# andreeaiana/manner

Measured on AMD Instinct MI355X. Metric: candidate news encoded+scored/sec, higher is better.
Workload: dtype f16; 1 GPU; configs[1]: CR-Module late fusion, MIND-small shape (65238-news pool), bert-base-uncased architectu~; modules=1, parallelism=dp1 (impressions sharded, no collective)

## Files before the change

### manner_amd/csrc/attention.hip

```cpp
#include <math.h>
#include <stdlib.h>

#include "common.h"

namespace manner {
namespace {

template <typename TE, int NKT>
__device__ __forceinline__ void attn_wave_bf16(const TE* __restrict__ qkv, TE* __restrict__ ctx,
                                               int tok0, int L, int H, int head, char* vl) {
  typedef typename E16<TE>::v8 e16x8;
  typedef typename E16<TE>::v4 e16x4;
  const int lane = threadIdx.x & 63, rr = lane & 31, h = lane >> 5;
  char* ol = vl + NKT * 32 * 128;
  const size_t ld = 3 * (size_t)H;
  const TE* Qb = qkv + (size_t)tok0 * ld + head * 64;
  const TE* Kb = Qb + H;
  const TE* Vb = Qb + 2 * H;

  const int r8 = lane >> 3, c8 = lane & 7;
  f32x4 kt_[NKT][4], qt_[4];
#pragma unroll
  for (int kt = 0; kt < NKT; ++kt)
#pragma unroll
// ... 874 lines not shown
        Row8<T>::load(Vb + (size_t)min(key, L - 1) * ld, vr);
#pragma unroll
        for (int e = 0; e < 8; ++e) o[e] = fmaf(p, vr[e], o[e]);
      }
    }
  }
  sum += __shfl_xor(sum, 8, 64); sum += __shfl_xor(sum, 16, 64); sum += __shfl_xor(sum, 32, 64);
#pragma unroll
  for (int e = 0; e < 8; ++e) {
    o[e] += __shfl_xor(o[e], 8, 64); o[e] += __shfl_xor(o[e], 16, 64); o[e] += __shfl_xor(o[e], 32, 64);
  }
  if (g == 0) {
    const float inv = 1.0f / sum;
#pragma unroll
    for (int e = 0; e < 8; ++e) o[e] *= inv;
    Row8<T>::store(dst, o);
  }
}

template <typename T>
__global__ __launch_bounds__(256) void attn_cls_kernel(const T* __restrict__ qcls, const T* __restrict__ kv,
                                                       T* __restrict__ ctx, const int32_t* __restrict__ cu,
                                                       int64_t n_pairs, int heads, int H) {
  const int64_t pair = (int64_t)blockIdx.x * 4 + (threadIdx.x >> 6);
  if (pair >= n_pairs) return;
  const int lane = threadIdx.x & 63, g = lane >> 3, c = lane & 7;
  const int n = (int)(pair / heads), head = (int)(pair - (int64_t)n * heads);
  const int tok0 = cu[n], L = cu[n + 1] - tok0;
  const size_t ld = 2 * (size_t)H;
  const T* Kb = kv + (size_t)tok0 * ld + head * 64 + 8 * c;
  const T* Vb = Kb + H;
  float q[8];
  Row8<T>::load(qcls + (size_t)n * H + head * 64 + 8 * c, q);
  if (L > MANNER_HIP_MAX_LEN) {
    attn_cls_long<T>(Kb, Vb, q, L, ld, g, ctx + (size_t)n * H + head * 64 + 8 * c);
    return;
  }
  constexpr int MAXR = MANNER_HIP_MAX_LEN / 8;
  float sc[MAXR];
  float mx = -INFINITY;
#pragma unroll
  for (int r = 0; r < MAXR; ++r) {
    const int key = 8 * r + g;
    float s = -INFINITY;
    if (8 * r < L) {
      float kr[8];
      Row8<T>::load(Kb + (size_t)min(key, L - 1) * ld, kr);
      float d = 0.f;
#pragma unroll
      for (int e = 0; e < 8; ++e) d = fmaf(q[e], kr[e], d);
      d += __shfl_xor(d, 1, 64); d += __shfl_xor(d, 2, 64); d += __shfl_xor(d, 4, 64);
      s = key < L ? d * 0.125f : -INFINITY;
    }
    sc[r] = s;
    mx = fmaxf(mx, s);
  }
  mx = fmaxf(mx, __shfl_xor(mx, 8, 64)); mx = fmaxf(mx, __shfl_xor(mx, 16, 64)); mx = fmaxf(mx, __shfl_xor(mx, 32, 64));
  float sum = 0.f, o[8] = {0.f, 0.f, 0.f, 0.f, 0.f, 0.f, 0.f, 0.f};
#pragma unroll
  for (int r = 0; r < MAXR; ++r) {
    if (8 * r < L) {
      const int key = 8 * r + g;
      const float p = expf(sc[r] - mx);
      sum += p;
      float vr[8];
      Row8<T>::load(Vb + (size_t)min(key, L - 1) * ld, vr);
#pragma unroll
      for (int e = 0; e < 8; ++e) o[e] = fmaf(p, vr[e], o[e]);
    }
  }
  sum += __shfl_xor(sum, 8, 64); sum += __shfl_xor(sum, 16, 64); sum += __shfl_xor(sum, 32, 64);
#pragma unroll
  for (int e = 0; e < 8; ++e) {
    o[e] += __shfl_xor(o[e], 8, 64); o[e] += __shfl_xor(o[e], 16, 64); o[e] += __shfl_xor(o[e], 32, 64);
  }
  if (g == 0) {
    const float inv = 1.0f / sum;
#pragma unroll
    for (int e = 0; e < 8; ++e) o[e] *= inv;
    Row8<T>::store(ctx + (size_t)n * H + head * 64 + 8 * c, o);
  }
}

}

int attention_cls(DType dt, const void* qcls, const void* kv, void* ctx_cls, const int32_t* cu, int64_t n_news, int heads,
                  int H, hipStream_t stream) {
  if (H != heads * 64) return fail(MANNER_HIP_E_INVALID, "head_dim must be 64 (H=%d heads=%d)", H, heads);
  const int64_t pairs = n_news * heads;
  dim3 g((unsigned)((pairs + 3) / 4)), b(256);
  if (dt == DT_BF16)
    hipLaunchKernelGGL(attn_cls_kernel<bf16_t>, g, b, 0, stream, static_cast<const bf16_t*>(qcls), static_cast<const bf16_t*>(kv),
                       static_cast<bf16_t*>(ctx_cls), cu, pairs, heads, H);
  else if (dt == DT_F16)
    hipLaunchKernelGGL(attn_cls_kernel<f16_t>, g, b, 0, stream, static_cast<const f16_t*>(qcls), static_cast<const f16_t*>(kv),
                       static_cast<f16_t*>(ctx_cls), cu, pairs, heads, H);
  else
    hipLaunchKernelGGL(attn_cls_kernel<float>, g, b, 0, stream, static_cast<const float*>(qcls), static_cast<const float*>(kv),
                       static_cast<float*>(ctx_cls), cu, pairs, heads, H);
  MANNER_LAUNCH_CHECK();
  return MANNER_HIP_OK;
}

static int attention_long(DType dt, const void* qkv, void* ctx, const int32_t* cu, int64_t pairs, int heads, int H, int max_len,
                          hipStream_t stream, void* split_out, DType split_dt) {
  if (is_16bit(dt)) {
    const int n_qb = (max_len + 32 * LONG16_WAVES - 1) / (32 * LONG16_WAVES);
    const int rows_cap = (max_len + 31) / 32 * 32;
    const int lds = rows_cap * 256 + LONG16_WAVES * 4096;
    static bool lds_raised_dev[MAX_DEVICES] = {};
    bool& lds_raised = lds_raised_dev[current_device_slot()];
    if (!lds_raised) {
      const int cap = MANNER_HIP_MAX_LEN_INFER * 256 + LONG16_WAVES * 4096;
      MANNER_HIP_TRY(hipFuncSetAttribute(reinterpret_cast<const void*>(attn_long16_kernel<bf16_t>), hipFuncAttributeMaxDynamicSharedMemorySize, cap));
      MANNER_HIP_TRY(hipFuncSetAttribute(reinterpret_cast<const void*>(attn_long16_kernel<f16_t>), hipFuncAttributeMaxDynamicSharedMemorySize, cap));
      lds_raised = true;
    }
    const dim3 grid((unsigned)(pairs * n_qb)), block(64 * LONG16_WAVES);
    if (dt == DT_F16)
      hipLaunchKernelGGL(attn_long16_kernel<f16_t>, grid, block, lds, stream, static_cast<const f16_t*>(qkv), static_cast<f16_t*>(ctx), cu,
                         pairs, n_qb, heads, H, rows_cap);
    else
      hipLaunchKernelGGL(attn_long16_kernel<bf16_t>, grid, block, lds, stream, static_cast<const bf16_t*>(qkv), static_cast<bf16_t*>(ctx), cu,
                         pairs, n_qb, heads, H, rows_cap);
  } else {
    const int n_qb = (max_len + 32 * LONGF_WAVES - 1) / (32 * LONGF_WAVES);
    static bool lds_raised_dev[MAX_DEVICES] = {};
    bool& lds_raised = lds_raised_dev[current_device_slot()];
    if (!lds_raised) {
      MANNER_HIP_TRY(hipFuncSetAttribute(reinterpret_cast<const void*>(attn_long_f32_kernel), hipFuncAttributeMaxDynamicSharedMemorySize, LONGF_LDS));
      lds_raised = true;
    }
    hipLaunchKernelGGL(attn_long_f32_kernel, dim3((unsigned)(pairs * n_qb)), dim3(64 * LONGF_WAVES), LONGF_LDS, stream,
                       static_cast<const float*>(qkv), static_cast<float*>(ctx), cu, pairs, n_qb, heads, H, split_out, (int)split_dt);
  }
  MANNER_LAUNCH_CHECK();
  return MANNER_HIP_OK;
}

int attention_varlen(DType dt, const void* qkv, void* ctx, const int32_t* cu, int64_t n_news, int heads, int H,
                     int max_len, hipStream_t stream, void* split_out, DType split_dt) {
  if (H != heads * 64) return fail(MANNER_HIP_E_INVALID, "head_dim must be 64 (H=%d heads=%d)", H, heads);
  if (max_len < 1 || max_len > MANNER_HIP_MAX_LEN_INFER)
    return fail(MANNER_HIP_E_INVALID, "padded length %d outside [1, %d]", max_len, MANNER_HIP_MAX_LEN_INFER);
  const int64_t pairs = n_news * heads;
  const bool long_rows = max_len > MANNER_HIP_MAX_LEN;
  const int short_len = long_rows ? MANNER_HIP_MAX_LEN : max_len;
  if (is_16bit(dt)) {
    const int nkt = (short_len + 31) / 32;
    const int lds_per_wave = nkt * 32 * 128 + 4096;
    static bool lds_raised_dev[MAX_DEVICES] = {};
    bool& lds_raised = lds_raised_dev[current_device_slot()];
    if (!lds_raised) {
      MANNER_HIP_TRY(hipFuncSetAttribute(reinterpret_cast<const void*>(attn_bf16_kernel<bf16_t>), hipFuncAttributeMaxDynamicSharedMemorySize, 4 * (4 * 32 * 128 + 4096)));
      MANNER_HIP_TRY(hipFuncSetAttribute(reinterpret_cast<const void*>(attn_bf16_kernel<f16_t>), hipFuncAttributeMaxDynamicSharedMemorySize, 4 * (4 * 32 * 128 + 4096)));
      lds_raised = true;
    }
    if (dt == DT_F16)
      hipLaunchKernelGGL(attn_bf16_kernel<f16_t>, dim3((unsigned)((pairs + 3) / 4)), dim3(256), 4 * lds_per_wave, stream,
                         static_cast<const f16_t*>(qkv), static_cast<f16_t*>(ctx), cu, pairs, heads, H, lds_per_wave);
    else
      hipLaunchKernelGGL(attn_bf16_kernel<bf16_t>, dim3((unsigned)((pairs + 3) / 4)), dim3(256), 4 * lds_per_wave, stream,
                         static_cast<const bf16_t*>(qkv), static_cast<bf16_t*>(ctx), cu, pairs, heads, H, lds_per_wave);
  } else {
    static const bool valu = getenv("MANNER_HIP_ATTN_F32_VALU") != nullptr;
    if (valu) {
// ... 39 lines not shown
```

### manner_amd/csrc/common.h

```cpp
#pragma once
#include <hip/hip_runtime.h>
#include <stddef.h>
#include <stdint.h>

#include "manner_hip.h"

typedef __bf16 bf16_t;
typedef __bf16 bf16x8 __attribute__((ext_vector_type(8)));
typedef __bf16 bf16x4 __attribute__((ext_vector_type(4)));
typedef _Float16 f16_t;
typedef _Float16 f16x8 __attribute__((ext_vector_type(8)));
typedef _Float16 f16x4 __attribute__((ext_vector_type(4)));
typedef short s16x4 __attribute__((ext_vector_type(4)));
typedef float f32x16 __attribute__((ext_vector_type(16)));
typedef float f32x4 __attribute__((ext_vector_type(4)));

#define LDS_PTR(p) ((__attribute__((address_space(3))) void*)(p))
#define GLOBAL_PTR(p) ((const __attribute__((address_space(1))) void*)(p))

namespace manner {

int fail(int code, const char* fmt, ...);

#define MANNER_HIP_TRY(expr)                                                            \
// ... 28 lines not shown
                EPI_GELU_GRAD = 9 ,
                EPI_BIAS_GELU_DUAL16 = 10 ,
                EPI_GELU_GRAD16 = 11  };
enum DType { DT_F32 = 0, DT_BF16 = 1, DT_F16 = 2 };
static inline bool is_16bit(DType d) { return d != DT_F32; }

template <typename T> struct E16;
template <> struct E16<bf16_t> {
  typedef bf16x8 v8; typedef bf16x4 v4;
  static constexpr DType dtype = DT_BF16;
  static __device__ __forceinline__ f32x4 mfma16(const v8& a, const v8& b, const f32x4& c) { return __builtin_amdgcn_mfma_f32_16x16x32_bf16(a, b, c, 0, 0, 0); }
  static __device__ __forceinline__ f32x16 mfma32(const v8& a, const v8& b, const f32x16& c) { return __builtin_amdgcn_mfma_f32_32x32x16_bf16(a, b, c, 0, 0, 0); }
};
template <> struct E16<f16_t> {
  typedef f16x8 v8; typedef f16x4 v4;
  static constexpr DType dtype = DT_F16;
  static __device__ __forceinline__ f32x4 mfma16(const v8& a, const v8& b, const f32x4& c) { return __builtin_amdgcn_mfma_f32_16x16x32_f16(a, b, c, 0, 0, 0); }
  static __device__ __forceinline__ f32x16 mfma32(const v8& a, const v8& b, const f32x16& c) { return __builtin_amdgcn_mfma_f32_32x32x16_f16(a, b, c, 0, 0, 0); }
};

int gemm_tn(DType in, DType out, Epilogue epi, const void* X, const void* W, const float* bias,
            const void* residual, void* Y, int64_t m_bound, int N, int K, const int* m_total,
            hipStream_t stream);

int gemm_tn_batched16(DType in, const void* X, const void* W, const float* bias, float* Y, int batch, int64_t xs, int64_t ws,
                      int64_t ys, int rows, int N, int K, const int* m_total, hipStream_t stream);

struct DlnFinalize { void* mr_out; int32_t* arrive; float eps; bool done; };
int gemm_tn_dln(DType dt, Epilogue epi, const void* X, const void* W, const float* bias, const float* vec, const void* mr,
                void* part, void* Y, int64_t m_bound, int N, int K, const int* m_total, hipStream_t stream, int64_t m_exact = -1,
                DlnFinalize* fin = nullptr);

int pool_logits_mfma(const float* x, const float* W, const float* bias, const float* query, int64_t R, int D, int Q,
                     float* logits, hipStream_t stream);

bool pool_fused_supported(int64_t B, int64_t S, int D, int Q);
size_t pool_fused_workspace_bytes(int D, int Q);
int pool_fused(const float* x, const float* W, const float* bias, const float* query, int64_t B, int64_t S, int D, int Q, float* out,
               void* workspace, size_t workspace_bytes, hipStream_t stream);

int lengths_and_offsets(const int64_t* mask, int64_t n_news, int64_t padded_len, int32_t* lens,
                        int32_t* cu , int32_t* m_total , int64_t m_bound,
                        int64_t expect_tokens, int32_t* status, hipStream_t stream, int max_len);
int embed_layernorm(DType out, const int64_t* ids, int64_t n_news, int64_t padded_len, const int32_t* cu,
                    const float* word, const float* pos, const float* type0, const float* gamma,
                    const float* beta, int H, float eps, int pos_offset, int vocab, int max_pos,
                    void* x, int32_t* status, hipStream_t stream);
int layernorm_rows(DType out, const float* pre, const float* gamma, const float* beta, int H, float eps,
                   void* x, int64_t m_bound, const int* m_total, hipStream_t stream);
int embed_raw(DType dt, const int64_t* ids, int64_t n_news, int64_t padded_len, const int32_t* cu, const float* word,
              const float* pos, const float* type0, int H, float eps, int pos_offset, int vocab, int max_pos,
              void* raw, void* mr, int32_t* status, hipStream_t stream);
__device__ __forceinline__ float2 dln_row_stats(const float2 (&v)[16], float inv_h, float eps) {
  float s1 = v[0].x, s2 = v[0].y;
#pragma unroll
  for (int g = 1; g < 16; ++g) { s1 += v[g].x; s2 += v[g].y; }
  const float mean = s1 * inv_h;
  const float var = fmaxf(fmaf(s2, inv_h, -(mean * mean)), 0.f);
  return float2{mean, 1.0f / sqrtf(var + eps)};
}
int dln_finalize(const void* part, int groups, int H, float eps, void* mr, int64_t m_bound, const int* m_total,
                 hipStream_t stream);
int gather_cls_ln(DType dt, const void* raw, const void* mr, const int32_t* cu, int64_t n_news, int H, const float* gamma,
                  const float* beta, void* dst, hipStream_t stream);
int fold_layernorm(DType dt, const float* w, const float* bias, const float* gamma, const float* beta, int N, int K, void* wf,
                   float* c1, float* c2, hipStream_t stream);
int scatter_hidden(DType in, DType out_dt, const void* x, const void* mr, const int32_t* cu, int64_t n_news, int64_t lp, int H,
                   const float* gamma, const float* beta, void* out, hipStream_t stream);
int split3_rows(DType dt, bool weight, const float* x, void* out, int K, int64_t rows, const int* m_total, hipStream_t stream);
int layernorm_rows_split(DType split_dt, const float* pre, const float* gamma, const float* beta, int H, float eps, float* x, void* a3,
                         int64_t m_bound, const int* m_total, hipStream_t stream);
int add_vectors(const float* a, const float* b, float* out, int n, hipStream_t stream);
int set_device_int(int32_t* p, int32_t value, hipStream_t stream);
int gather_cls(DType in, const void* x, const int32_t* cu, int64_t n_news, int H, float* out, hipStream_t stream);
int gather_cls_rows(DType dt, const void* x, const int32_t* cu, int64_t n_news, int H, void* dst, hipStream_t stream);
int convert_f32_to_16(DType dt, const float* src, void* dst, int64_t n, hipStream_t stream);

int attention_varlen(DType dt, const void* qkv, void* ctx, const int32_t* cu, int64_t n_news, int heads,
                     int H, int max_len, hipStream_t stream, void* split_out = nullptr, DType split_dt = DT_F32);

int attention_cls(DType dt, const void* qcls, const void* kv, void* ctx_cls, const int32_t* cu, int64_t n_news,
                  int heads, int H, hipStream_t stream);

}
```

### manner_amd/csrc/encoder.hip

```cpp
#include <stdarg.h>
#include <stdio.h>
#include <stdlib.h>

#include <vector>

#include "common.h"

namespace manner {

static thread_local char g_err[512] = "";

int fail(int code, const char* fmt, ...) {
  va_list ap;
  va_start(ap, fmt);
  vsnprintf(g_err, sizeof(g_err), fmt, ap);
  va_end(ap);
  return code;
}

struct LayerWeights {
  void* wqkv = nullptr;
  void* wo = nullptr;
  void* w1 = nullptr;
  void* w2 = nullptr;
  void* wqkv_f = nullptr;
  void* w1_f = nullptr;
  float *cq1 = nullptr, *cf1 = nullptr;
};
struct LayerParams {
  float *bqkv, *bo, *ln1g, *ln1b, *b1, *b2, *ln2g, *ln2b;
  float *cq2 = nullptr, *cf2 = nullptr, *bo_res = nullptr, *b2_res = nullptr;
};

}

struct manner_hip_encoder {
  manner_hip_encoder_config cfg;
  uint32_t precisions = 0;
  float *word = nullptr, *pos = nullptr, *type0 = nullptr, *embg = nullptr, *embb = nullptr;
  std::vector<manner::LayerParams> params;
  std::vector<manner::LayerWeights> w[5];
  int32_t* status = nullptr;
  static constexpr int ARRIVE_CAP = 4096;
  int32_t* arrive = nullptr;
  std::vector<void*> allocs;
  int n_streams = 2;
  bool defer_ln = false;
  static constexpr int MAX_STREAMS = 4;
  hipStream_t side[MAX_STREAMS] = {};
  hipEvent_t join_ev[MAX_STREAMS] = {};
  hipEvent_t phase_ev[MAX_STREAMS] = {};
  bool profiling = false;
  struct Span { hipEvent_t a, b; int cls; };
  std::vector<Span> spans;
  std::vector<hipEvent_t> free_events;
};

namespace manner {
namespace {

inline DType act_dtype(int prec) { return prec == MANNER_HIP_PREC_BF16 ? DT_BF16 : prec == MANNER_HIP_PREC_F16 ? DT_F16 : DT_F32; }
inline size_t act_bytes(int prec) { return (prec == MANNER_HIP_PREC_BF16 || prec == MANNER_HIP_PREC_F16) ? 2 : 4; }
inline bool is_x3(int prec) { return prec == MANNER_HIP_PREC_BF16X3 || prec == MANNER_HIP_PREC_F16X3; }
inline DType x3_dtype(int prec) { return prec == MANNER_HIP_PREC_F16X3 ? DT_F16 : DT_BF16; }

int dev_alloc(manner_hip_encoder* e, size_t bytes, void** out) {
  MANNER_HIP_TRY(hipMalloc(out, bytes));
  e->allocs.push_back(*out);
  return MANNER_HIP_OK;
}
int dev_copy_f32(manner_hip_encoder* e, const float* src, size_t n, float** out, hipStream_t s) {
  int rc = dev_alloc(e, n * sizeof(float), (void**)out);
  if (rc) return rc;
  MANNER_HIP_TRY(hipMemcpyAsync(*out, src, n * sizeof(float), hipMemcpyDeviceToDevice, s));
  return MANNER_HIP_OK;
}
int pack_matrix(int prec, const float* src, size_t n, void* dst, size_t elem_off, hipStream_t s) {
  if (prec == MANNER_HIP_PREC_BF16 || prec == MANNER_HIP_PREC_F16)
    return convert_f32_to_16(prec == MANNER_HIP_PREC_F16 ? DT_F16 : DT_BF16, src, static_cast<char*>(dst) + elem_off * 2, (int64_t)n, s);
  MANNER_HIP_TRY(hipMemcpyAsync(static_cast<float*>(dst) + elem_off, src, n * sizeof(float), hipMemcpyDeviceToDevice, s));
  return MANNER_HIP_OK;
}

struct ProfScope {
  manner_hip_encoder* e; hipStream_t s; hipEvent_t a = nullptr, b = nullptr; int cls;
  static hipEvent_t get(manner_hip_encoder* e) {
    hipEvent_t ev = nullptr;
    if (!e->free_events.empty()) { ev = e->free_events.back(); e->free_events.pop_back(); }
    else if (hipEventCreate(&ev) != hipSuccess) ev = nullptr;
    return ev;
  }
  ProfScope(manner_hip_encoder* enc, hipStream_t st, int c) : e(enc), s(st), cls(c) {
    if (!e->profiling) return;
    a = get(e); b = get(e);
    if (a && b) (void)hipEventRecord(a, s);
  }
  ~ProfScope() {
    if (!a || !b) return;
    (void)hipEventRecord(b, s);
    e->spans.push_back({a, b, cls});
  }
};

struct Workspace {
  int32_t *lens, *cu, *m_total;
  float* pre;
  void *x, *qkv, *ctx, *ffn;
  void *xcls, *qcls;
  void *mr_in, *mr_mid, *part;
  int32_t* arrive = nullptr;
  void* a3;
  void* a3h;
  void *acc_x, *acc_ctx, *acc_x1;
  int32_t* cls_total;
  int64_t cls_cap;
};

constexpr int64_t CLS_CAP = 16384;

size_t carve(const manner_hip_encoder* e, int64_t max_news, int64_t m_cap, int prec, char* base, Workspace* ws) {
  const size_t es = act_bytes(prec);
  const size_t H = e->cfg.hidden, I = e->cfg.intermediate;
  size_t off = 0;
  if (ws) { ws->a3 = nullptr; ws->a3h = nullptr; }
  auto take = [&](size_t bytes) { size_t o = off; off += (size_t)round_up((int64_t)bytes, 256); return base ? base + o : nullptr; };
  char* p;
  p = take((size_t)max_news * 4); if (ws) ws->lens = (int32_t*)p;
  p = take((size_t)(max_news + 1) * 4); if (ws) ws->cu = (int32_t*)p;
  p = take(256); if (ws) ws->m_total = (int32_t*)p;
  p = take((size_t)m_cap * H * 4); if (ws) ws->pre = (float*)p;
  p = take((size_t)m_cap * H * es); if (ws) ws->x = p;
  p = take((size_t)m_cap * 3 * H * es); if (ws) ws->qkv = p;
  p = take((size_t)m_cap * H * es); if (ws) ws->ctx = p;
  p = take((size_t)m_cap * I * es); if (ws) ws->ffn = p;
  const size_t n_pad = (size_t)round_up(max_news, 256);
  p = take(n_pad * H * es); if (ws) ws->xcls = p;
  p = take(n_pad * H * es); if (ws) ws->qcls = p;
  p = take((size_t)m_cap * 8); if (ws) ws->mr_in = p;
  p = take((size_t)m_cap * 8); if (ws) ws->mr_mid = p;
  p = take((size_t)m_cap * (H / 64) * 8); if (ws) ws->part = p;
  if (is_x3(prec)) {
    p = take((size_t)m_cap * 3 * (H > I ? H : I) * 2); if (ws) ws->a3 = p;
    p = take((size_t)m_cap * 3 * H * 2); if (ws) ws->a3h = p;
  }
  const int64_t cls_cap = m_cap < CLS_CAP ? m_cap : CLS_CAP;
  if (ws) ws->cls_cap = cls_cap;
  p = take((size_t)(cls_cap + 256) * H * es); if (ws) ws->acc_x = p;
  p = take((size_t)(cls_cap + 256) * H * es); if (ws) ws->acc_ctx = p;
  p = take((size_t)(cls_cap + 256) * H * es); if (ws) ws->acc_x1 = p;
  p = take(256); if (ws) ws->cls_total = (int32_t*)p;
  return off;
}

struct PhaseGuard {
  hipEvent_t ev; hipStream_t s; bool done = false;
  void mark() { if (ev && !done) { (void)hipEventRecord(ev, s); done = true; } }
  ~PhaseGuard() { mark(); }
};

int encode_chunk(manner_hip_encoder* e, const int64_t* ids, const int64_t* mask, int64_t n_news, int64_t lp,
                 int64_t m_bound, int64_t expect_tokens, int prec, void* out, const Workspace& ws, hipStream_t s,
                 hipEvent_t phase_mark = nullptr, int hidden_layers = -1, DType hidden_dt = DT_F32, int64_t cls_off = 0) {
  PhaseGuard phase{phase_mark, s};
  const manner_hip_encoder_config& c = e->cfg;
  const DType dt = act_dtype(prec);
  const int H = c.hidden, I = c.intermediate;
  int rc;
  {
    ProfScope ps(e, s, MANNER_HIP_PROF_LENGTHS);
    if ((rc = lengths_and_offsets(mask, n_news, lp, ws.lens, ws.cu, ws.m_total, m_bound, expect_tokens, e->status, s,
                                 MANNER_HIP_MAX_LEN_INFER))) return rc;
  }
  const int pos_offset = c.arch == MANNER_HIP_ARCH_ROBERTA ? c.pad_id + 1 : 0;
#define PROF_STEP(cls, call) { ProfScope ps(e, s, cls); if ((rc = (call))) return rc; }
  const size_t es = act_bytes(prec);
  if (is_16bit(dt) && e->defer_ln) {
    PROF_STEP(MANNER_HIP_PROF_EMBED, embed_raw(dt, ids, n_news, lp, ws.cu, e->word, e->pos, e->type0, H, c.ln_eps, pos_offset,
                                               c.vocab, c.max_pos, ws.x, ws.mr_in, e->status, s))
    const int groups = H / 64;
    for (int l = 0; l < c.layers; ++l) {
      const LayerWeights& w = e->w[prec][l];
      const LayerParams& p = e->params[l];
      const float* g_in = l == 0 ? e->embg : e->params[l - 1].ln2g;
      const float* b_in = l == 0 ? e->embb : e->params[l - 1].ln2b;
      if (l == hidden_layers) break;
      if (hidden_layers < 0 && l + 1 == c.layers) {
        const int64_t n_bound = round_up(n_news, 256);
        const int32_t* n_total = ws.m_total + 1;
        const char* wkv = static_cast<const char*>(w.wqkv_f) + (size_t)H * H * 2;
        PROF_STEP(MANNER_HIP_PROF_GEMM_QKV, gemm_tn_dln(dt, EPI_NORM, ws.x, wkv, p.cq2 + H, w.cq1 + H, ws.mr_in, nullptr, ws.qkv, m_bound, 2 * H, H, ws.m_total, s, expect_tokens))
        char* ax = static_cast<char*>(ws.acc_x) + (size_t)cls_off * H * es;
        char* actx = static_cast<char*>(ws.acc_ctx) + (size_t)cls_off * H * es;
        PROF_STEP(MANNER_HIP_PROF_GATHER, gather_cls_ln(dt, ws.x, ws.mr_in, ws.cu, n_news, H, g_in, b_in, ax, s))
        PROF_STEP(MANNER_HIP_PROF_CLS_TAIL, gemm_tn(dt, dt, EPI_BIAS, ax, w.wqkv, p.bqkv, nullptr, ws.qcls, n_bound, H, H, n_total, s))
        PROF_STEP(MANNER_HIP_PROF_ATTENTION, attention_cls(dt, ws.qcls, ws.qkv, actx, ws.cu, n_news, c.heads, H, s))
        break;
      }
      PROF_STEP(MANNER_HIP_PROF_GEMM_QKV, gemm_tn_dln(dt, EPI_NORM, ws.x, w.wqkv_f, p.cq2, w.cq1, ws.mr_in, nullptr, ws.qkv, m_bound, 3 * H, H, ws.m_total, s, expect_tokens))
      PROF_STEP(MANNER_HIP_PROF_ATTENTION, attention_varlen(dt, ws.qkv, ws.ctx, ws.cu, n_news, c.heads, H, (int)lp, s))
      const bool fan_in = ws.arrive && m_bound / 192 + 1 <= manner_hip_encoder::ARRIVE_CAP;
      DlnFinalize fin_mid{ws.mr_mid, fan_in ? ws.arrive : nullptr, c.ln_eps, false}, fin_in{ws.mr_in, fan_in ? ws.arrive : nullptr, c.ln_eps, false};
      PROF_STEP(MANNER_HIP_PROF_GEMM_OUT, gemm_tn_dln(dt, EPI_NRES, ws.ctx, w.wo, p.bo_res, g_in, ws.mr_in, ws.part, ws.x, m_bound, H, H, ws.m_total, s, expect_tokens, &fin_mid))
      if (!fin_mid.done) PROF_STEP(MANNER_HIP_PROF_LAYERNORM, dln_finalize(ws.part, groups, H, c.ln_eps, ws.mr_mid, m_bound, ws.m_total, s))
      if (l == 0) phase.mark();
      PROF_STEP(MANNER_HIP_PROF_GEMM_FFN1, gemm_tn_dln(dt, EPI_NORM_GELU, ws.x, w.w1_f, p.cf2, w.cf1, ws.mr_mid, nullptr, ws.ffn, m_bound, I, H, ws.m_total, s, expect_tokens))
      PROF_STEP(MANNER_HIP_PROF_GEMM_FFN2, gemm_tn_dln(dt, EPI_NRES, ws.ffn, w.w2, p.b2_res, p.ln1g, ws.mr_mid, ws.part, ws.x, m_bound, H, I, ws.m_total, s, expect_tokens, &fin_in))
      if (!fin_in.done) PROF_STEP(MANNER_HIP_PROF_LAYERNORM, dln_finalize(ws.part, groups, H, c.ln_eps, ws.mr_in, m_bound, ws.m_total, s))
    }
    if (hidden_layers >= 0) {
      const float* g = hidden_layers == 0 ? e->embg : e->params[hidden_layers - 1].ln2g;
      const float* b = hidden_layers == 0 ? e->embb : e->params[hidden_layers - 1].ln2b;
      PROF_STEP(MANNER_HIP_PROF_GATHER, scatter_hidden(dt, hidden_dt, ws.x, ws.mr_in, ws.cu, n_news, lp, H, g, b, out, s))
    }
    return MANNER_HIP_OK;
  }
  {
    ProfScope ps(e, s, MANNER_HIP_PROF_EMBED);
    if ((rc = embed_layernorm(dt, ids, n_news, lp, ws.cu, e->word, e->pos, e->type0, e->embg, e->embb, H, c.ln_eps,
                              pos_offset, c.vocab, c.max_pos, ws.x, e->status, s)))
      return rc;
  }
  const bool x3 = is_x3(prec);
  const DType xdt = x3_dtype(prec);
  auto gemm = [&](DType out_dt, Epilogue epi, const void* A, const void* Wm, const float* bias, const void* res, void* Y,
                  int64_t mb, int N, int K, const int* mt) -> int {
    if (!x3) return gemm_tn(dt, out_dt, epi, A, Wm, bias, res, Y, mb, N, K, mt, s);
    int r = split3_rows(xdt, false, static_cast<const float*>(A), ws.a3, K, mb, mt, s);
    if (r) return r;
    return gemm_tn(xdt, DT_F32, epi == EPI_BIAS_RES ? EPI_BIAS_RES_F32 : epi, ws.a3, Wm, bias, res, Y, mb, N, 3 * K, mt, s);
  };
  const int full_layers = hidden_layers >= 0 ? hidden_layers : c.layers - 1;
  if (x3) PROF_STEP(MANNER_HIP_PROF_LAYERNORM, split3_rows(xdt, false, static_cast<const float*>(ws.x), ws.a3h, H, m_bound, ws.m_total, s))
  for (int l = 0; l < full_layers && x3; ++l) {
    const LayerWeights& w = e->w[prec][l];
    const LayerParams& p = e->params[l];
    float* xf = static_cast<float*>(ws.x);
    PROF_STEP(MANNER_HIP_PROF_GEMM_QKV, gemm_tn(xdt, DT_F32, EPI_BIAS, ws.a3h, w.wqkv, p.bqkv, nullptr, ws.qkv, m_bound, 3 * H, 3 * H, ws.m_total, s))
    static const bool attn_valu = getenv("MANNER_HIP_ATTN_F32_VALU") != nullptr;
    if (attn_valu) {
      PROF_STEP(MANNER_HIP_PROF_ATTENTION, attention_varlen(dt, ws.qkv, ws.ctx, ws.cu, n_news, c.heads, H, (int)lp, s))
      PROF_STEP(MANNER_HIP_PROF_LAYERNORM, split3_rows(xdt, false, static_cast<const float*>(ws.ctx), ws.a3h, H, m_bound, ws.m_total, s))
    } else {
      PROF_STEP(MANNER_HIP_PROF_ATTENTION, attention_varlen(dt, ws.qkv, ws.ctx, ws.cu, n_news, c.heads, H, (int)lp, s, ws.a3h, xdt))
    }
    PROF_STEP(MANNER_HIP_PROF_GEMM_OUT, gemm_tn(xdt, DT_F32, EPI_BIAS_RES_F32, ws.a3h, w.wo, p.bo, ws.x, ws.pre, m_bound, H, 3 * H, ws.m_total, s))
    PROF_STEP(MANNER_HIP_PROF_LAYERNORM, layernorm_rows_split(xdt, ws.pre, p.ln1g, p.ln1b, H, c.ln_eps, xf, ws.a3h, m_bound, ws.m_total, s))
    if (l == 0) phase.mark();
    PROF_STEP(MANNER_HIP_PROF_GEMM_FFN1, gemm_tn(xdt, xdt, EPI_BIAS_GELU_SPLIT3, ws.a3h, w.w1, p.b1, nullptr, ws.a3, m_bound, I, 3 * H, ws.m_total, s))
    PROF_STEP(MANNER_HIP_PROF_GEMM_FFN2, gemm_tn(xdt, DT_F32, EPI_BIAS_RES_F32, ws.a3, w.w2, p.b2, ws.x, ws.pre, m_bound, H, 3 * I, ws.m_total, s))
    PROF_STEP(MANNER_HIP_PROF_LAYERNORM, layernorm_rows_split(xdt, ws.pre, p.ln2g, p.ln2b, H, c.ln_eps, xf, ws.a3h, m_bound, ws.m_total, s))
  }
  for (int l = 0; l < full_layers && !x3; ++l) {
    const LayerWeights& w = e->w[prec][l];
    const LayerParams& p = e->params[l];
    PROF_STEP(MANNER_HIP_PROF_GEMM_QKV, gemm(dt, EPI_BIAS, ws.x, w.wqkv, p.bqkv, nullptr, ws.qkv, m_bound, 3 * H, H, ws.m_total))
    PROF_STEP(MANNER_HIP_PROF_ATTENTION, attention_varlen(dt, ws.qkv, ws.ctx, ws.cu, n_news, c.heads, H, (int)lp, s))
    PROF_STEP(MANNER_HIP_PROF_GEMM_OUT, gemm(DT_F32, EPI_BIAS_RES, ws.ctx, w.wo, p.bo, ws.x, ws.pre, m_bound, H, H, ws.m_total))
    PROF_STEP(MANNER_HIP_PROF_LAYERNORM, layernorm_rows(dt, ws.pre, p.ln1g, p.ln1b, H, c.ln_eps, ws.x, m_bound, ws.m_total, s))
    if (l == 0) phase.mark();
    PROF_STEP(MANNER_HIP_PROF_GEMM_FFN1, gemm(dt, EPI_BIAS_GELU, ws.x, w.w1, p.b1, nullptr, ws.ffn, m_bound, I, H, ws.m_total))
    PROF_STEP(MANNER_HIP_PROF_GEMM_FFN2, gemm(DT_F32, EPI_BIAS_RES, ws.ffn, w.w2, p.b2, ws.x, ws.pre, m_bound, H, I, ws.m_total))
    PROF_STEP(MANNER_HIP_PROF_LAYERNORM, layernorm_rows(dt, ws.pre, p.ln2g, p.ln2b, H, c.ln_eps, ws.x, m_bound, ws.m_total, s))
  }
  if (hidden_layers >= 0) {
    PROF_STEP(MANNER_HIP_PROF_GATHER, scatter_hidden(dt, hidden_dt, ws.x, nullptr, ws.cu, n_news, lp, H, nullptr, nullptr, out, s))
    return MANNER_HIP_OK;
  }
  {
    const LayerWeights& w = e->w[prec][c.layers - 1];
    const LayerParams& p = e->params[c.layers - 1];
    const int64_t n_bound = round_up(n_news, 256);
    const int32_t* n_total = ws.m_total + 1;
    const char* wkv = static_cast<const char*>(w.wqkv) + (size_t)H * (x3 ? (size_t)3 * H * 2 : (size_t)H * es);
    if (x3)
      PROF_STEP(MANNER_HIP_PROF_GEMM_QKV, gemm_tn(xdt, DT_F32, EPI_BIAS, ws.a3h, wkv, p.bqkv + H, nullptr, ws.qkv, m_bound, 2 * H, 3 * H, ws.m_total, s))
// ... 126 lines not shown
  e->precisions = precisions;
  int rc = MANNER_HIP_OK;
  auto guard = [&](int r) { if (r && !rc) rc = r; return r == 0; };
  const size_t HH = (size_t)H * H, HI = (size_t)H * I;
  do {
    if (!guard(dev_copy_f32(e, weights[MANNER_HIP_W_WORD_EMB], (size_t)cfg->vocab * H, &e->word, s))) break;
    if (!guard(dev_copy_f32(e, weights[MANNER_HIP_W_POS_EMB], (size_t)cfg->max_pos * H, &e->pos, s))) break;
    if (!guard(dev_copy_f32(e, weights[MANNER_HIP_W_TYPE_EMB], (size_t)H, &e->type0, s))) break;
    if (!guard(dev_copy_f32(e, weights[MANNER_HIP_W_EMB_LN_G], H, &e->embg, s))) break;
    if (!guard(dev_copy_f32(e, weights[MANNER_HIP_W_EMB_LN_B], H, &e->embb, s))) break;
    if (!guard(dev_alloc(e, 256, (void**)&e->status))) break;
    if (hipMemsetAsync(e->status, 0, 256, s) != hipSuccess) { rc = fail(MANNER_HIP_E_RUNTIME, "memset failed"); break; }
    const size_t arrive_bytes = (size_t)manner_hip_encoder::MAX_STREAMS * manner_hip_encoder::ARRIVE_CAP * sizeof(int32_t);
    if (!guard(dev_alloc(e, arrive_bytes, (void**)&e->arrive))) break;
    if (hipMemsetAsync(e->arrive, 0, arrive_bytes, s) != hipSuccess) { rc = fail(MANNER_HIP_E_RUNTIME, "memset failed"); break; }
    if (const char* ev = getenv("MANNER_HIP_STREAMS")) {
      const int v = atoi(ev);
      e->n_streams = v < 1 ? 1 : (v > manner_hip_encoder::MAX_STREAMS ? manner_hip_encoder::MAX_STREAMS : v);
    }
    e->defer_ln = (precisions & ((1u << MANNER_HIP_PREC_BF16) | (1u << MANNER_HIP_PREC_F16))) && H % 256 == 0 && I % 256 == 0;
    if (const char* ev = getenv("MANNER_HIP_DEFER_LN")) e->defer_ln = e->defer_ln && atoi(ev) != 0;
    for (int i = 0; i < e->n_streams && !rc; ++i) {
      if ((i > 0 && hipStreamCreateWithFlags(&e->side[i], hipStreamNonBlocking) != hipSuccess) ||
          hipEventCreateWithFlags(&e->join_ev[i], hipEventDisableTiming) != hipSuccess ||
          hipEventCreateWithFlags(&e->phase_ev[i], hipEventDisableTiming) != hipSuccess)
        rc = fail(MANNER_HIP_E_RUNTIME, "encoder_create: side stream/event creation failed");
    }
    if (rc) break;
    e->params.resize(L);
    for (int p = 0; p < 5; ++p) if (precisions & (1u << p)) e->w[p].resize(L);
    for (int l = 0; l < L && !rc; ++l) {
      const float* const* wl = weights + MANNER_HIP_W_EMB_COUNT + l * MANNER_HIP_WL_COUNT;
      LayerParams& P = e->params[l];
      if (!guard(dev_alloc(e, 3 * (size_t)H * 4, (void**)&P.bqkv))) break;
      for (int j = 0; j < 3; ++j)
        if (hipMemcpyAsync(P.bqkv + j * H, wl[MANNER_HIP_WL_Q_B + 2 * j], H * 4, hipMemcpyDeviceToDevice, s) != hipSuccess) rc = fail(MANNER_HIP_E_RUNTIME, "bias copy failed");
      guard(dev_copy_f32(e, wl[MANNER_HIP_WL_AO_B], H, &P.bo, s));
      guard(dev_copy_f32(e, wl[MANNER_HIP_WL_ALN_G], H, &P.ln1g, s));
      guard(dev_copy_f32(e, wl[MANNER_HIP_WL_ALN_B], H, &P.ln1b, s));
      guard(dev_copy_f32(e, wl[MANNER_HIP_WL_FF1_B], I, &P.b1, s));
      guard(dev_copy_f32(e, wl[MANNER_HIP_WL_FF2_B], H, &P.b2, s));
      guard(dev_copy_f32(e, wl[MANNER_HIP_WL_OLN_G], H, &P.ln2g, s));
      guard(dev_copy_f32(e, wl[MANNER_HIP_WL_OLN_B], H, &P.ln2b, s));
      for (int p = 0; p < 4 && !rc; ++p) {
        if (is_x3(p) || !(precisions & (1u << p))) continue;
        const size_t es = act_bytes(p);
        LayerWeights& W = e->w[p][l];
        if (!guard(dev_alloc(e, 3 * HH * es, &W.wqkv))) break;
        if (!guard(dev_alloc(e, HH * es, &W.wo))) break;
        if (!guard(dev_alloc(e, HI * es, &W.w1))) break;
        if (!guard(dev_alloc(e, HI * es, &W.w2))) break;
        for (int j = 0; j < 3; ++j) guard(pack_matrix(p, wl[MANNER_HIP_WL_Q_W + 2 * j], HH, W.wqkv, j * HH, s));
        guard(pack_matrix(p, wl[MANNER_HIP_WL_AO_W], HH, W.wo, 0, s));
        guard(pack_matrix(p, wl[MANNER_HIP_WL_FF1_W], HI, W.w1, 0, s));
        guard(pack_matrix(p, wl[MANNER_HIP_WL_FF2_W], HI, W.w2, 0, s));
      }
      for (int p : {MANNER_HIP_PREC_BF16X3, MANNER_HIP_PREC_F16X3}) {
        if (!(precisions & (1u << p)) || rc) continue;
        const DType sdt = x3_dtype(p);
        LayerWeights& W = e->w[p][l];
        if (!guard(dev_alloc(e, 3 * HH * 6, &W.wqkv)) || !guard(dev_alloc(e, HH * 6, &W.wo)) ||
            !guard(dev_alloc(e, HI * 6, &W.w1)) || !guard(dev_alloc(e, HI * 6, &W.w2))) break;
        for (int j = 0; j < 3; ++j)
          guard(split3_rows(sdt, true, wl[MANNER_HIP_WL_Q_W + 2 * j], static_cast<char*>(W.wqkv) + (size_t)j * HH * 6, H, H, nullptr, s));
        guard(split3_rows(sdt, true, wl[MANNER_HIP_WL_AO_W], W.wo, H, H, nullptr, s));
        guard(split3_rows(sdt, true, wl[MANNER_HIP_WL_FF1_W], W.w1, H, I, nullptr, s));
        guard(split3_rows(sdt, true, wl[MANNER_HIP_WL_FF2_W], W.w2, I, H, nullptr, s));
      }
      if (e->defer_ln && !rc) {
        const float* g_in = l == 0 ? e->embg : e->params[l - 1].ln2g;
        const float* b_in = l == 0 ? e->embb : e->params[l - 1].ln2b;
        if (!guard(dev_alloc(e, 3 * (size_t)H * 4, (void**)&P.cq2)) || !guard(dev_alloc(e, (size_t)I * 4, (void**)&P.cf2))) break;
        if (!guard(dev_alloc(e, (size_t)H * 4, (void**)&P.bo_res)) || !guard(dev_alloc(e, (size_t)H * 4, (void**)&P.b2_res))) break;
        for (int p : {MANNER_HIP_PREC_BF16, MANNER_HIP_PREC_F16}) {
          if (!(precisions & (1u << p)) || rc) continue;
          const DType fdt = act_dtype(p);
          LayerWeights& W = e->w[p][l];
          if (!guard(dev_alloc(e, 3 * HH * 2, &W.wqkv_f)) || !guard(dev_alloc(e, HI * 2, &W.w1_f))) break;
          if (!guard(dev_alloc(e, 3 * (size_t)H * 4, (void**)&W.cq1)) || !guard(dev_alloc(e, (size_t)I * 4, (void**)&W.cf1))) break;
          for (int j = 0; j < 3; ++j)
            guard(fold_layernorm(fdt, wl[MANNER_HIP_WL_Q_W + 2 * j], wl[MANNER_HIP_WL_Q_B + 2 * j], g_in, b_in, H, H,
                                 static_cast<char*>(W.wqkv_f) + j * HH * 2, W.cq1 + j * H, P.cq2 + j * H, s));
          guard(fold_layernorm(fdt, wl[MANNER_HIP_WL_FF1_W], wl[MANNER_HIP_WL_FF1_B], P.ln1g, P.ln1b, I, H, W.w1_f, W.cf1, P.cf2, s));
        }
        guard(add_vectors(P.bo, b_in, P.bo_res, H, s));
        guard(add_vectors(P.b2, P.ln1b, P.b2_res, H, s));
      }
    }
    if (rc) break;
    if (hipStreamSynchronize(s) != hipSuccess) { rc = fail(MANNER_HIP_E_RUNTIME, "encoder_create: stream sync failed: %s", hipGetErrorString(hipGetLastError())); break; }
  } while (0);
  if (rc) { manner_hip_encoder_destroy(e); return rc; }
  *out = e;
  return MANNER_HIP_OK;
}

size_t manner_hip_encoder_workspace_bytes(manner_hip_encoder_t enc, int64_t max_news, int64_t max_tokens, int32_t precision) {
  if (!enc || max_news <= 0 || max_tokens <= 0 || precision < 0 || precision > 4) return 0;
  return enc->n_streams * carve(enc, max_news, round_up(max_tokens, 256), precision, nullptr, nullptr);
}

static int encode_impl(manner_hip_encoder_t enc, const int64_t* ids, const int64_t* mask, const int32_t* host_lengths,
                       int64_t n_news, int64_t padded_len, int32_t precision, void* out, void* workspace,
                       size_t workspace_bytes, manner_hip_stream_t stream, int hidden_layers, DType hidden_dt) {
  if (!enc) return fail(MANNER_HIP_E_INVALID, "encode_cls: null handle");
  if (n_news == 0) return MANNER_HIP_OK;
  if (!ids || !mask || !out || !workspace || n_news < 0) return fail(MANNER_HIP_E_INVALID, "encode_cls: null pointer");
  if (precision < 0 || precision > 4 || !(enc->precisions & (1u << precision))) return fail(MANNER_HIP_E_INVALID, "encode_cls: precision %d was not requested at encoder_create", precision);
  if (padded_len < 1 || padded_len > MANNER_HIP_MAX_LEN_INFER) return fail(MANNER_HIP_E_INVALID, "encode_cls: padded_len %lld outside [1, %d]", (long long)padded_len, MANNER_HIP_MAX_LEN_INFER);
  if ((uintptr_t)workspace % 256) return fail(MANNER_HIP_E_INVALID, "encode_cls: workspace must be 256-byte aligned");
  const int H = enc->cfg.hidden;
  const int ns = enc->profiling ? 1 : enc->n_streams;
  const size_t ws_each = (workspace_bytes / enc->n_streams) / 256 * 256;
  const size_t es = act_bytes(precision);
  const size_t per_tok = (size_t)H * 4 + ((size_t)5 * H + enc->cfg.intermediate) * es +
                         (is_x3(precision) ? (size_t)6 * (H > enc->cfg.intermediate ? H : enc->cfg.intermediate) + (size_t)6 * H : 0);
  int64_t m_cap = (int64_t)(ws_each / per_tok) / 256 * 256;
  int64_t n_cap = 0;
  while (m_cap >= 256) {
    n_cap = m_cap;
    if (n_cap > n_news) n_cap = n_news;
    if (carve(enc, n_cap, m_cap, precision, nullptr, nullptr) <= ws_each) break;
    m_cap -= 256;
  }
  if (m_cap < 256 || m_cap < padded_len) return fail(MANNER_HIP_E_WORKSPACE, "encode_cls: workspace of %zu bytes cannot hold one 256-token tile per stream", workspace_bytes);
  Workspace ws[manner_hip_encoder::MAX_STREAMS];
  for (int i = 0; i < ns; ++i) {
    carve(enc, n_cap, m_cap, precision, static_cast<char*>(workspace) + i * ws_each, &ws[i]);
    ws[i].arrive = enc->arrive + (size_t)i * manner_hip_encoder::ARRIVE_CAP;
  }
  hipStream_t s0 = (hipStream_t)stream;
  int forked = 0;
  auto join = [&]() -> int {
    for (int i = 1; i <= forked; ++i) {
      MANNER_HIP_TRY(hipEventRecord(enc->join_ev[i], enc->side[i]));
      MANNER_HIP_TRY(hipStreamWaitEvent(s0, enc->join_ev[i], 0));
    }
    forked = 0;
    return MANNER_HIP_OK;
  };
  struct Chunk { int64_t n0, cnt, m_bound, expect; };
  std::vector<Chunk> plan;
  for (int64_t n0 = 0; n0 < n_news;) {
    int64_t cnt = 0, m_bound, expect = -1;
    if (host_lengths) {
      int64_t tok = 0;
      while (n0 + cnt < n_news && cnt < n_cap) {
        const int64_t len = host_lengths[n0 + cnt];
        if (len < 1 || len > padded_len)
          return fail(MANNER_HIP_E_INVALID, "encode_cls: host_lengths[%lld]=%lld outside [1, padded_len]", (long long)(n0 + cnt), (long long)len);
        if (tok + len > m_cap) break;
        tok += len;
        ++cnt;
      }
      m_bound = round_up(tok, 256);
      expect = tok;
    } else {
      cnt = m_cap / padded_len;
      if (cnt > n_cap) cnt = n_cap;
      if (cnt > n_news - n0) cnt = n_news - n0;
      m_bound = round_up(cnt * padded_len, 256);
    }
    plan.push_back({n0, cnt, m_bound, expect});
    n0 += cnt;
  }
  const int n_chunks = (int)plan.size();
// ... 85 lines not shown
```

Baseline: 45540 candidates/s.

## Fold last-layer CLS attention through key/value weights to skip full K/V projection

For the final encoder layer, where only the [CLS] output is needed, the K/V projection GEMM over every token is skipped. Instead each CLS query is pushed back through the key weights (pre-scaled by the LayerNorm gamma), scores are computed directly against the normalised hidden states, and the attention-weighted input sums are projected through the value weights afterwards. This replaces an O(tokens·2H·H) GEMM with per-news work that scales with heads·H·tokens, plus a small values GEMM. The path is on by default for f16 and can be toggled with an environment variable. It adds precision risk, since the folded query vectors are rounded to 16-bit, and it needs a workspace-size condition to hold.

```diff
diff --git a/manner_amd/csrc/attention.hip b/manner_amd/csrc/attention.hip
--- a/manner_amd/csrc/attention.hip
+++ b/manner_amd/csrc/attention.hip
@@ -980,6 +980,274 @@
   }
 }
 
+constexpr int FOLD_MAX_LEN = MANNER_HIP_MAX_LEN_INFER;
+
+template <typename T, int NC>
+__global__ __launch_bounds__(256) void attn_cls_fold_kernel(const T* __restrict__ x, const float2* __restrict__ mr,
+                                                            const int32_t* __restrict__ cu, const float* __restrict__ gamma,
+                                                            const float* __restrict__ beta, float* au) {
+  constexpr int H = 256 * NC, HEADS = 4 * NC, KP = H / 64, HR = HEADS / 2;
+  typedef typename E16<T>::v8 v8;
+  typedef typename E16<T>::v4 v4;
+  __shared__ __attribute__((aligned(16))) float S[FOLD_MAX_LEN * 16];
+  __shared__ float2 mr_s[FOLD_MAX_LEN];
+  __shared__ float red_m[4][16], red_s[4][16];
+  static_assert(HR * H <= FOLD_MAX_LEN * 16, "the partial sums of half the heads reuse the score table");
+  const int n = blockIdx.x, tid = threadIdx.x, wave = tid >> 6, lane = tid & 63, r = lane & 15, g = lane >> 4;
+  const int tok0 = cu[n];
+  const int L = min(max(cu[n + 1] - tok0, 0), FOLD_MAX_LEN);
+  float* aun = au + (size_t)n * HEADS * H;
+  const T* xn = x + (size_t)tok0 * H;
+
+  v8 afr[KP][2];
+  float asum = 0.f;
+#pragma unroll
+  for (int q = 0; q < KP; ++q) {
+    f32x4 f[4] = {};
+    if (r < HEADS) {
+#pragma unroll
+      for (int e = 0; e < 4; ++e) f[e] = *reinterpret_cast<const f32x4*>(aun + (size_t)r * H + q * 64 + g * 16 + 4 * e);
+    }
+#pragma unroll
+    for (int i = 0; i < 8; ++i) {
+      const T lo = (T)f[i >> 2][i & 3], hi = (T)f[2 + (i >> 2)][i & 3];
+      afr[q][0][i] = lo;
+      afr[q][1][i] = hi;
+      asum += (float)lo + (float)hi;
+    }
+  }
+  asum += __shfl_xor(asum, 16, 64); asum += __shfl_xor(asum, 32, 64);
+  float A4[4];
+#pragma unroll
+  for (int i = 0; i < 4; ++i) A4[i] = __shfl(asum, 4 * g + i, 64);
+
+  for (int t0 = wave * 16; t0 < L; t0 += 64) {
+    const int t = t0 + r, tc = min(t, L - 1);
+    const T* row = xn + (size_t)tc * H + g * 16;
+    const float2 ms = mr[tok0 + tc];
+    f32x4 acc = {0.f, 0.f, 0.f, 0.f};
+#pragma unroll
+    for (int q = 0; q < KP; ++q) {
+      const v8 b0 = *reinterpret_cast<const v8*>(row + q * 64), b1 = *reinterpret_cast<const v8*>(row + q * 64 + 8);
+      acc = E16<T>::mfma16(afr[q][0], b0, acc);
+      acc = E16<T>::mfma16(afr[q][1], b1, acc);
+    }
+    if (t < L) {
+      f32x4 s;
+#pragma unroll
+      for (int i = 0; i < 4; ++i) s[i] = ms.y * (acc[i] - ms.x * A4[i]) * 0.125f;
+      *reinterpret_cast<f32x4*>(&S[t * 16 + 4 * g]) = s;
+      if (g == 0) mr_s[t] = ms;
+    }
+  }
+  __syncthreads();
+
+  {
+    const int h = tid & 15, stripe = tid >> 4;
+    float m = -INFINITY;
+    for (int t = stripe; t < L; t += 16) m = fmaxf(m, S[t * 16 + h]);
+    m = fmaxf(m, __shfl_xor(m, 16, 64)); m = fmaxf(m, __shfl_xor(m, 32, 64));
+    if (lane < 16) red_m[wave][lane] = m;
+    __syncthreads();
+    m = fmaxf(fmaxf(red_m[0][h], red_m[1][h]), fmaxf(red_m[2][h], red_m[3][h]));
+    float sum = 0.f;
+    for (int t = stripe; t < L; t += 16) {
+      const float e = expf(S[t * 16 + h] - m);
+      S[t * 16 + h] = e;
+      sum += e;
+    }
+    sum += __shfl_xor(sum, 16, 64); sum += __shfl_xor(sum, 32, 64);
+    if (lane < 16) red_s[wave][lane] = sum;
+    __syncthreads();
+    sum = (red_s[0][h] + red_s[1][h]) + (red_s[2][h] + red_s[3][h]);
+    const float inv = sum > 0.f ? 1.0f / sum : 0.f;
+    for (int t = stripe; t < L; t += 16) S[t * 16 + h] *= inv * mr_s[t].y;
+  }
+  __syncthreads();
+
+  float acc[HEADS][4 * NC];
+#pragma unroll
+  for (int h = 0; h < HEADS; ++h)
+#pragma unroll
+    for (int k = 0; k < 4 * NC; ++k) acc[h][k] = 0.f;
+  {
+    v4 cur[NC], nxt[NC];
+    const T* col = xn + lane * 4;
+    if (wave < L) {
+#pragma unroll
+      for (int c = 0; c < NC; ++c) cur[c] = *reinterpret_cast<const v4*>(col + (size_t)wave * H + c * 256);
+    }
+    for (int t = wave; t < L; t += 4) {
+      if (t + 4 < L) {
+#pragma unroll
+        for (int c = 0; c < NC; ++c) nxt[c] = *reinterpret_cast<const v4*>(col + (size_t)(t + 4) * H + c * 256);
+      }
+      const float mu = mr_s[t].x;
+      float wt[HEADS], xm[4 * NC];
+#pragma unroll
+      for (int c = 0; c < NC; ++c) {
+        const f32x4 w4 = *reinterpret_cast<const f32x4*>(&S[t * 16 + 4 * c]);
+#pragma unroll
+        for (int e = 0; e < 4; ++e) { wt[4 * c + e] = w4[e]; xm[4 * c + e] = (float)cur[c][e] - mu; }
+      }
+#pragma unroll
+      for (int h = 0; h < HEADS; ++h)
+#pragma unroll
+        for (int k = 0; k < 4 * NC; ++k) acc[h][k] = fmaf(wt[h], xm[k], acc[h][k]);
+#pragma unroll
+      for (int c = 0; c < NC; ++c) cur[c] = nxt[c];
+    }
+  }
+  __syncthreads();
+
+#pragma unroll
+  for (int half = 0; half < 2; ++half) {
+#pragma unroll
+    for (int w = 0; w < 4; ++w) {
+      if (wave == w) {
+#pragma unroll
+        for (int hh = 0; hh < HR; ++hh)
+#pragma unroll
+          for (int c = 0; c < NC; ++c) {
+            float* p = &S[hh * H + c * 256 + lane * 4];
+            f32x4 v = {acc[half * HR + hh][4 * c], acc[half * HR + hh][4 * c + 1], acc[half * HR + hh][4 * c + 2], acc[half * HR + hh][4 * c + 3]};
+            if (w > 0) {
+              const f32x4 o = *reinterpret_cast<const f32x4*>(p);
+#pragma unroll
+              for (int e = 0; e < 4; ++e) v[e] = o[e] + v[e];
+            }
+            if (w < 3) {
+              *reinterpret_cast<f32x4*>(p) = v;
+            } else {
+              const f32x4 g4 = *reinterpret_cast<const f32x4*>(gamma + c * 256 + lane * 4);
+              const f32x4 b4 = *reinterpret_cast<const f32x4*>(beta + c * 256 + lane * 4);
+#pragma unroll
+              for (int e = 0; e < 4; ++e) v[e] = fmaf(g4[e], v[e], b4[e]);
+              *reinterpret_cast<f32x4*>(aun + (size_t)(half * HR + hh) * H + c * 256 + lane * 4) = v;
+            }
+          }
+      }
+      __syncthreads();
+    }
+  }
+}
+
+template <typename T>
+__global__ __launch_bounds__(256) void cls_fold_keys_kernel(const T* __restrict__ qcls, const T* __restrict__ wkt, float* __restrict__ a,
+                                                            int64_t n_news, int heads, int H) {
+  typedef typename E16<T>::v8 v8;
+  const int h = blockIdx.y, wave = threadIdx.x >> 6, lane = threadIdx.x & 63, r = lane & 15, g = lane >> 4;
+  const int64_t n = (int64_t)blockIdx.x * 16 + r, nn = n < n_news ? n : n_news - 1;
+  const T* qp = qcls + (size_t)nn * H + h * 64 + g * 16;
+  const v8 q0 = *reinterpret_cast<const v8*>(qp), q1 = *reinterpret_cast<const v8*>(qp + 8);
+  const int tiles = H / 64;
+  for (int i = 0; i < tiles; ++i) {
+    const int j0 = (wave * tiles + i) * 16;
+    const T* wp = wkt + (size_t)(j0 + r) * H + h * 64 + g * 16;
+    const v8 w0 = *reinterpret_cast<const v8*>(wp), w1 = *reinterpret_cast<const v8*>(wp + 8);
+    f32x4 acc = {0.f, 0.f, 0.f, 0.f};
+    acc = E16<T>::mfma16(w0, q0, acc);
+    acc = E16<T>::mfma16(w1, q1, acc);
+    if (n < n_news) *reinterpret_cast<f32x4*>(a + ((size_t)n * heads + h) * H + j0 + 4 * g) = acc;
+  }
+}
+
+template <typename T>
+__global__ __launch_bounds__(256) void cls_fold_values_kernel(const float* __restrict__ u, const T* __restrict__ wv, const float* __restrict__ bv,
+                                                              T* __restrict__ ctx, int64_t n_news, int heads, int H) {
+  typedef typename E16<T>::v8 v8;
+  typedef typename E16<T>::v4 v4;
+  const int h = blockIdx.y, wave = threadIdx.x >> 6, lane = threadIdx.x & 63, r = lane & 15, g = lane >> 4;
+  const int64_t n = (int64_t)blockIdx.x * 16 + r, nn = n < n_news ? n : n_news - 1;
+  const T* wp = wv + (size_t)(h * 64 + wave * 16 + r) * H + g * 16;
+  const float* up = u + ((size_t)nn * heads + h) * H + g * 16;
+  f32x4 acc = {0.f, 0.f, 0.f, 0.f};
+  for (int q = 0; q < H / 64; ++q) {
+    const v8 w0 = *reinterpret_cast<const v8*>(wp + q * 64), w1 = *reinterpret_cast<const v8*>(wp + q * 64 + 8);
+    f32x4 f[4];
+#pragma unroll
+    for (int e = 0; e < 4; ++e) f[e] = *reinterpret_cast<const f32x4*>(up + q * 64 + 4 * e);
+    v8 u0, u1;
+#pragma unroll
+    for (int i = 0; i < 8; ++i) { u0[i] = (T)f[i >> 2][i & 3]; u1[i] = (T)f[2 + (i >> 2)][i & 3]; }
+    acc = E16<T>::mfma16(w0, u0, acc);
+    acc = E16<T>::mfma16(w1, u1, acc);
+  }
+  if (n < n_news) {
+    const int d = h * 64 + wave * 16 + 4 * g;
+    const f32x4 b = *reinterpret_cast<const f32x4*>(bv + d);
+    v4 o;
+#pragma unroll
+    for (int i = 0; i < 4; ++i) o[i] = (T)(acc[i] + b[i]);
+    *reinterpret_cast<v4*>(ctx + (size_t)n * H + d) = o;
+  }
+}
+
+template <typename T>
+__global__ __launch_bounds__(256) void cls_fold_pack_keys_kernel(const float* __restrict__ wk, const float* __restrict__ gamma, int H,
+                                                                 T* __restrict__ wkt) {
+  const int j = blockIdx.x;
+  const float gj = gamma[j];
+  for (int d = threadIdx.x; d < H; d += 256) wkt[(size_t)j * H + d] = (T)(gj * wk[(size_t)d * H + j]);
+}
+
+}
+
+int cls_fold_pack_keys(DType dt, const float* wk, const float* gamma, int H, void* wkt, hipStream_t stream) {
+  if (dt == DT_F16)
+    hipLaunchKernelGGL(cls_fold_pack_keys_kernel<f16_t>, dim3((unsigned)H), dim3(256), 0, stream, wk, gamma, H, static_cast<f16_t*>(wkt));
+  else
+    hipLaunchKernelGGL(cls_fold_pack_keys_kernel<bf16_t>, dim3((unsigned)H), dim3(256), 0, stream, wk, gamma, H, static_cast<bf16_t*>(wkt));
+  MANNER_LAUNCH_CHECK();
+  return MANNER_HIP_OK;
+}
+
+static int cls_fold_check(DType dt, int64_t n_news, int heads, int H) {
+  if (!is_16bit(dt) || H != heads * 64 || H % 256 || H > 1024 || n_news < 1)
+    return fail(MANNER_HIP_E_INVALID, "folded [CLS] attention: 16-bit, head_dim 64, H %% 256 == 0, H <= 1024 (H=%d heads=%d)", H, heads);
+  return MANNER_HIP_OK;
+}
+
+int cls_fold_keys(DType dt, const void* qcls, const void* wkt, float* a, int64_t n_news, int heads, int H, hipStream_t stream) {
+  if (int rc = cls_fold_check(dt, n_news, heads, H)) return rc;
+  const dim3 grid((unsigned)((n_news + 15) / 16), (unsigned)heads), block(256);
+  if (dt == DT_F16)
+    hipLaunchKernelGGL(cls_fold_keys_kernel<f16_t>, grid, block, 0, stream, static_cast<const f16_t*>(qcls), static_cast<const f16_t*>(wkt), a, n_news, heads, H);
+  else
+    hipLaunchKernelGGL(cls_fold_keys_kernel<bf16_t>, grid, block, 0, stream, static_cast<const bf16_t*>(qcls), static_cast<const bf16_t*>(wkt), a, n_news, heads, H);
+  MANNER_LAUNCH_CHECK();
+  return MANNER_HIP_OK;
+}
+
+int cls_fold_values(DType dt, const float* u, const void* wv, const float* bv, void* ctx_cls, int64_t n_news, int heads, int H,
+                    hipStream_t stream) {
+  if (int rc = cls_fold_check(dt, n_news, heads, H)) return rc;
+  const dim3 grid((unsigned)((n_news + 15) / 16), (unsigned)heads), block(256);
+  if (dt == DT_F16)
+    hipLaunchKernelGGL(cls_fold_values_kernel<f16_t>, grid, block, 0, stream, u, static_cast<const f16_t*>(wv), bv, static_cast<f16_t*>(ctx_cls), n_news, heads, H);
+  else
+    hipLaunchKernelGGL(cls_fold_values_kernel<bf16_t>, grid, block, 0, stream, u, static_cast<const bf16_t*>(wv), bv, static_cast<bf16_t*>(ctx_cls), n_news, heads, H);
+  MANNER_LAUNCH_CHECK();
+  return MANNER_HIP_OK;
+}
+
+int attention_cls_fold(DType dt, const void* x, const void* mr, const int32_t* cu, int64_t n_news, int heads, int H, const float* gamma,
+                       const float* beta, float* au, hipStream_t stream) {
+  if (int rc = cls_fold_check(dt, n_news, heads, H)) return rc;
+  const dim3 grid((unsigned)n_news), block(256);
+  const float2* mrp = static_cast<const float2*>(mr);
+#define MANNER_CLS_FOLD(T_, NC_) \
+  hipLaunchKernelGGL((attn_cls_fold_kernel<T_, NC_>), grid, block, 0, stream, static_cast<const T_*>(x), mrp, cu, gamma, beta, au)
+  if (dt == DT_F16) {
+    switch (H / 256) { case 1: MANNER_CLS_FOLD(f16_t, 1); break; case 2: MANNER_CLS_FOLD(f16_t, 2); break;
+                       case 3: MANNER_CLS_FOLD(f16_t, 3); break; default: MANNER_CLS_FOLD(f16_t, 4); }
+  } else {
+    switch (H / 256) { case 1: MANNER_CLS_FOLD(bf16_t, 1); break; case 2: MANNER_CLS_FOLD(bf16_t, 2); break;
+                       case 3: MANNER_CLS_FOLD(bf16_t, 3); break; default: MANNER_CLS_FOLD(bf16_t, 4); }
+  }
+#undef MANNER_CLS_FOLD
+  MANNER_LAUNCH_CHECK();
+  return MANNER_HIP_OK;
 }
 
 int attention_cls(DType dt, const void* qcls, const void* kv, void* ctx_cls, const int32_t* cu, int64_t n_news, int heads,
diff --git a/manner_amd/csrc/common.h b/manner_amd/csrc/common.h
--- a/manner_amd/csrc/common.h
+++ b/manner_amd/csrc/common.h
@@ -134,4 +134,11 @@
 int attention_cls(DType dt, const void* qcls, const void* kv, void* ctx_cls, const int32_t* cu, int64_t n_news,
                   int heads, int H, hipStream_t stream);
 
+int cls_fold_pack_keys(DType dt, const float* wk, const float* gamma, int H, void* wkt, hipStream_t stream);
+int cls_fold_keys(DType dt, const void* qcls, const void* wkt, float* a, int64_t n_news, int heads, int H, hipStream_t stream);
+int attention_cls_fold(DType dt, const void* x, const void* mr, const int32_t* cu, int64_t n_news, int heads, int H, const float* gamma,
+                       const float* beta, float* au, hipStream_t stream);
+int cls_fold_values(DType dt, const float* u, const void* wv, const float* bv, void* ctx_cls, int64_t n_news, int heads, int H,
+                    hipStream_t stream);
+
 }
diff --git a/manner_amd/csrc/encoder.hip b/manner_amd/csrc/encoder.hip
--- a/manner_amd/csrc/encoder.hip
+++ b/manner_amd/csrc/encoder.hip
@@ -25,6 +25,7 @@
   void* w2 = nullptr;
   void* wqkv_f = nullptr;
   void* w1_f = nullptr;
+  void* wk_t = nullptr;
   float *cq1 = nullptr, *cf1 = nullptr;
 };
 struct LayerParams {
@@ -187,10 +188,22 @@
       if (hidden_layers < 0 && l + 1 == c.layers) {
         const int64_t n_bound = round_up(n_news, 256);
         const int32_t* n_total = ws.m_total + 1;
+        char* ax = static_cast<char*>(ws.acc_x) + (size_t)cls_off * H * es;
+        char* actx = static_cast<char*>(ws.acc_ctx) + (size_t)cls_off * H * es;
+        const char* fold_env = getenv("MANNER_HIP_CLS_FOLD");
+        const bool fold = w.wk_t && (fold_env ? atoi(fold_env) != 0 : dt == DT_F16) &&
+                          (size_t)n_news * c.heads * H * 4 <= (size_t)m_bound * 3 * H * es;
+        if (fold) {
+          float* au = static_cast<float*>(ws.qkv);
+          PROF_STEP(MANNER_HIP_PROF_GATHER, gather_cls_ln(dt, ws.x, ws.mr_in, ws.cu, n_news, H, g_in, b_in, ax, s))
+          PROF_STEP(MANNER_HIP_PROF_CLS_TAIL, gemm_tn(dt, dt, EPI_BIAS, ax, w.wqkv, p.bqkv, nullptr, ws.qcls, n_bound, H, H, n_total, s))
+          PROF_STEP(MANNER_HIP_PROF_CLS_TAIL, cls_fold_keys(dt, ws.qcls, w.wk_t, au, n_news, c.heads, H, s))
+          PROF_STEP(MANNER_HIP_PROF_ATTENTION, attention_cls_fold(dt, ws.x, ws.mr_in, ws.cu, n_news, c.heads, H, g_in, b_in, au, s))
+          PROF_STEP(MANNER_HIP_PROF_CLS_TAIL, cls_fold_values(dt, au, static_cast<const char*>(w.wqkv) + (size_t)2 * H * H * es, p.bqkv + 2 * H, actx, n_news, c.heads, H, s))
+          break;
+        }
         const char* wkv = static_cast<const char*>(w.wqkv_f) + (size_t)H * H * 2;
         PROF_STEP(MANNER_HIP_PROF_GEMM_QKV, gemm_tn_dln(dt, EPI_NORM, ws.x, wkv, p.cq2 + H, w.cq1 + H, ws.mr_in, nullptr, ws.qkv, m_bound, 2 * H, H, ws.m_total, s, expect_tokens))
-        char* ax = static_cast<char*>(ws.acc_x) + (size_t)cls_off * H * es;
-        char* actx = static_cast<char*>(ws.acc_ctx) + (size_t)cls_off * H * es;
         PROF_STEP(MANNER_HIP_PROF_GATHER, gather_cls_ln(dt, ws.x, ws.mr_in, ws.cu, n_news, H, g_in, b_in, ax, s))
         PROF_STEP(MANNER_HIP_PROF_CLS_TAIL, gemm_tn(dt, dt, EPI_BIAS, ax, w.wqkv, p.bqkv, nullptr, ws.qcls, n_bound, H, H, n_total, s))
         PROF_STEP(MANNER_HIP_PROF_ATTENTION, attention_cls(dt, ws.qcls, ws.qkv, actx, ws.cu, n_news, c.heads, H, s))
@@ -483,6 +496,10 @@
             guard(fold_layernorm(fdt, wl[MANNER_HIP_WL_Q_W + 2 * j], wl[MANNER_HIP_WL_Q_B + 2 * j], g_in, b_in, H, H,
                                  static_cast<char*>(W.wqkv_f) + j * HH * 2, W.cq1 + j * H, P.cq2 + j * H, s));
           guard(fold_layernorm(fdt, wl[MANNER_HIP_WL_FF1_W], wl[MANNER_HIP_WL_FF1_B], P.ln1g, P.ln1b, I, H, W.w1_f, W.cf1, P.cf2, s));
+          if (l + 1 == L) {
+            if (!guard(dev_alloc(e, HH * 2, &W.wk_t))) break;
+            guard(cls_fold_pack_keys(fdt, wl[MANNER_HIP_WL_K_W], g_in, H, W.wk_t, s));
+          }
         }
         guard(add_vectors(P.bo, b_in, P.bo_res, H, s));
         guard(add_vectors(P.b2, P.ln1b, P.b2_res, H, s));
```

Measured after the change: 45870 candidates/s (median of 6 runs). About the same (+0.7%).
